# wildminder/ComfyUI-KEEP

Hardware: AMD Instinct MI355X
Metric: restored 512x512 face frames/sec, T=20 clip (higher is better)
Workload: dtype f16x3; 1 GPU; 48 independent clips x T=20 x 512x512 per GPU (BASELINE configs[1] clips), KEEP config, synthetic weights seed 0, precision policy x3; clips_per_gpu=48, clip_length=20, parallelism=dp1 over clips, precision_policy=x3

## Files before the change

### comfyui-keep_amd/csrc/keep_attn.hip

```cpp
#include <math.h>
#include <stdlib.h>

#include <type_traits>

#include "keep_common.h"
#include "../../include/keep_cv_hip.h"

static constexpr int KEEP_NT_ATTN_O = 0;


struct AttnP {
  const float* q;
  const float* k;
  const float* v;
  const unsigned short* q16;
  const unsigned short* k16;
  const unsigned short* v16;
  float* o;
  long q_bs, q_ts, q_hs, k_bs, k_ts, k_hs, v_bs, v_ts, v_hs, o_bs, o_ts, o_hs;
  int B, H, Lq, Lk, D, Dv;
  float scale;
  int mode, T, seg_len;
  int img_h, img_w, ksplit, shift, kv_rot, n_img;
  int nslices;
// ... 235 lines not shown
        if (t < p.Lk) kreg[u] = *reinterpret_cast<const float4*>(p.k + kv_offset(p, b, t, p.k_bs, p.k_ts) + kh + c);
      }
      if (i < 32 * vc4n) {
        const int row = i / vc4n, c = (i - row * vc4n) << 2;
        const int t = kt * 32 + row;
        if (t < p.Lk && dv0 + c < p.Dv)
          vreg[u] = *reinterpret_cast<const float4*>(p.v + kv_offset(p, b, t, p.v_bs, p.v_ts) + vh + dv0 + c);
      }
    }
  };
  auto pf_commit = [&]() {
#pragma unroll
    for (int u = 0; u < PF; ++u) {
      const int i = tid + u * NT;
      if (i < 32 * kc4n) {
        const int row = i / kc4n, c = (i - row * kc4n) << 2;
        float* d = Ks + row * QP + c;
        d[0] = kreg[u].x; d[1] = kreg[u].y; d[2] = kreg[u].z; d[3] = kreg[u].w;
      }
      if (i < 32 * vc4n) {
        const int row = i / vc4n, c = (i - row * vc4n) << 2;
        *reinterpret_cast<float4*>(Vs + row * DVS + c) = vreg[u];
      }
    }
  };

  if (prefetch) {
    pf_issue(0);
    pf_commit();
  }

  for (int kt = 0; kt < ntiles; ++kt) {
    f32x16 s;
#pragma unroll
    for (int r = 0; r < 16; ++r) s[r] = 0.f;

    if (prefetch) {
      __syncthreads();
      if (kt + 1 < ntiles) pf_issue(kt + 1);
      for (int d2 = 0; d2 < DC; d2 += 2) s = __builtin_amdgcn_mfma_f32_32x32x2f32(kp[d2], qp[d2], s, 0, 0, 0);
    } else {
      for (int ch = 0; ch < nch; ++ch) {
        __syncthreads();
        if (nch > 1)
          load_tile_direct<NT, true>(p, p.q, p.q_bs, p.q_ts, qh, b, q0, p.Lq, WAVES * 32, ch * DC, DC, p.D, Qs, QP,
                                     tid, qk_vec);
        load_tile_direct<NT, false>(p, p.k, p.k_bs, p.k_ts, kh, b, kt * 32, p.Lk, 32, ch * DC, DC, p.D, Ks, QP, tid,
                                    qk_vec);
        if (ch == 0)
          load_tile_direct<NT, false>(p, p.v, p.v_bs, p.v_ts, vh, b, kt * 32, p.Lk, 32, dv0, DVS, p.Dv, Vs, DVS, tid,
                                      v_vec);
        __syncthreads();
        for (int d2 = 0; d2 < DC; d2 += 2) s = __builtin_amdgcn_mfma_f32_32x32x2f32(kp[d2], qp[d2], s, 0, 0, 0);
      }
    }

    float mloc = -INFINITY;
#pragma unroll
    for (int r = 0; r < 16; ++r) {
      const int key = kt * 32 + (r & 3) + 8 * (r >> 2) + 4 * lhi;
      float val = s[r] * p.scale;
      if (p.mode == 2 && p.shift > 0 && key < p.Lk) {
        if (win_region(p, b, key) != my_region) val += -100.0f;
      }
      if (key >= p.Lk) val = -INFINITY;
      s[r] = val;
      mloc = fmaxf(mloc, val);
    }
    mloc = fmaxf(mloc, __shfl_xor(mloc, 32));
    const float m_new = fmaxf(m_run, mloc);
    const float alpha = expf(m_run - m_new);
    float lsum = 0.f;
#pragma unroll
    for (int r = 0; r < 16; ++r) {
      const float pv = expf(s[r] - m_new);
      s[r] = pv;
      lsum += pv;
    }
    lsum += __shfl_xor(lsum, 32);
    l_run = l_run * alpha + lsum;
    m_run = m_new;

#pragma unroll
    for (int r = 0; r < 16; ++r) {
      const int qrow = (r & 3) + 8 * (r >> 2) + 4 * lhi;
      const float ar = __shfl(alpha, qrow);
#pragma unroll
      for (int j = 0; j < DVT; ++j) o[j][r] *= ar;
    }
#pragma unroll
    for (int r = 0; r < 16; ++r) {
      const int krow = (r & 3) + 8 * (r >> 2) + 4 * lhi;
      const float* vp = Vs + krow * DVS + l31;
#pragma unroll
      for (int j = 0; j < DVT; ++j) o[j] = __builtin_amdgcn_mfma_f32_32x32x2f32(s[r], vp[j * 32], o[j], 0, 0, 0);
    }
    if (prefetch && kt + 1 < ntiles) {
      __syncthreads();
      pf_commit();
    }
  }

  const float inv_l = 1.0f / l_run;
#pragma unroll
  for (int r = 0; r < 16; ++r) {
    const int qrow = (r & 3) + 8 * (r >> 2) + 4 * lhi;
    const float il = __shfl(inv_l, qrow);
    const int t = q0 + wave * 32 + qrow;
    if (t < p.Lq) {
      const long base = q_offset(p, b, t, p.o_bs, p.o_ts) + (long)head * p.o_hs;
#pragma unroll
      for (int j = 0; j < DVT; ++j) {
        const int dv = dv0 + j * 32 + l31;
        if (dv < p.Dv) p.o[base + dv] = o[j][r] * il;
      }
    }
  }
}

template <int WAVES, int DVT>
static int launch_attn(const AttnP& p, const AttnPlan& pl, hipStream_t st) {
  const int rc = keep_raise_lds_limit<attn_f32_kernel<WAVES, DVT>>("keep_attention");
  if (rc != KEEP_OK) return rc;
  dim3 grid(cdiv(p.Lq, WAVES * 32), p.H * p.nslices, p.B);
  hipLaunchKernelGGL((attn_f32_kernel<WAVES, DVT>), grid, dim3(64 * WAVES), pl.lds, st, p);
  KEEP_LAUNCH_CHECK("keep_attention");
  return KEEP_OK;
}

typedef __attribute__((ext_vector_type(8))) __bf16 abf16x8;

__device__ __forceinline__ int vt_pos(int key) {
  return (((key >> 4) << 1) + ((key >> 2) & 1)) * 8 + ((((key >> 3) & 1) << 2) | (key & 3));
}

template <int WAVES, int DVT>
__global__ __launch_bounds__(64 * WAVES) void attn_bf16_kernel(AttnP p) {
  extern __shared__ __attribute__((aligned(16))) __bf16 smem16[];
  constexpr int DVS = DVT * 32;
  constexpr int NT = 64 * WAVES;
  constexpr int VP = 40;
  const int DC = p.D < 128 ? p.D : 128;
  const int nch = p.D / DC;
  const int QP = DC + 8;
  __bf16* Qs = smem16;
  __bf16* Ks = Qs + WAVES * 32 * QP;
  __bf16* Vt = Ks + 32 * QP;

  const int tid = threadIdx.x;
  const int lane = tid & 63;
  const int wave = tid >> 6;
  const int l31 = lane & 31, lhi = lane >> 5;
  const int b = blockIdx.z;
  const int head = blockIdx.y / p.nslices;
  const int dv0 = (blockIdx.y - head * p.nslices) * DVS;
  const int q0 = blockIdx.x * (WAVES * 32);
  const long qh = (long)head * p.q_hs, kh = (long)head * p.k_hs, vh = (long)head * p.v_hs;
  const int g8n = DC >> 3;

  auto stage_rows = [&](const float* base, long bs, long ts, long hoff, bool is_q, int t0, int tmax, int nrows,
                        int c0, __bf16* dst) {
    for (int i = tid; i < nrows * g8n; i += NT) {
      const int row = i / g8n, c = (i - row * g8n) << 3;
      const int t = t0 + row;
      abf16x8 h;
      if (t < tmax) {
        const float* src = base + (is_q ? q_offset(p, b, t, bs, ts) : kv_offset(p, b, t, bs, ts)) + hoff + c0 + c;
        const float4 a = *reinterpret_cast<const float4*>(src);
        const float4 c4 = *reinterpret_cast<const float4*>(src + 4);
        h[0] = (__bf16)a.x; h[1] = (__bf16)a.y; h[2] = (__bf16)a.z; h[3] = (__bf16)a.w;
        h[4] = (__bf16)c4.x; h[5] = (__bf16)c4.y; h[6] = (__bf16)c4.z; h[7] = (__bf16)c4.w;
      } else {
#pragma unroll
        for (int j = 0; j < 8; ++j) h[j] = (__bf16)0.f;
      }
      *reinterpret_cast<abf16x8*>(dst + row * QP + c) = h;
    }
  };
  auto stage_vt = [&](int kt) {
    for (int i = tid; i < 16 * DVS; i += NT) {
      const int pair = i / DVS, dv = i - pair * DVS;
      const int k0 = pair * 2;
      const int t = kt * 32 + k0;
      float v0 = 0.f, v1 = 0.f;
      if (dv0 + dv < p.Dv) {
        if (t < p.Lk) v0 = p.v[kv_offset(p, b, t, p.v_bs, p.v_ts) + vh + dv0 + dv];
        if (t + 1 < p.Lk) v1 = p.v[kv_offset(p, b, t + 1, p.v_bs, p.v_ts) + vh + dv0 + dv];
      }
      __bf16* d = Vt + dv * VP + vt_pos(k0);
      d[0] = (__bf16)v0;
      d[1] = (__bf16)v1;
    }
  };

  if (nch == 1) stage_rows(p.q, p.q_bs, p.q_ts, qh, true, q0, p.Lq, WAVES * 32, 0, Qs);

  const int my_q = q0 + wave * 32 + l31;
  int my_region = 0;
  if (p.mode == 2 && p.shift > 0 && my_q < p.Lq) my_region = win_region(p, b, my_q);

  float m_run = -INFINITY, l_run = 0.f;
  f32x16 o[DVT];
#pragma unroll
  for (int j = 0; j < DVT; ++j)
#pragma unroll
    for (int r = 0; r < 16; ++r) o[j][r] = 0.f;

  const __bf16* kp = Ks + l31 * QP + lhi * 8;
  const __bf16* qp = Qs + (wave * 32 + l31) * QP + lhi * 8;
  const int ntiles = (p.Lk + 31) / 32;

  for (int kt = 0; kt < ntiles; ++kt) {
    f32x16 s;
#pragma unroll
    for (int r = 0; r < 16; ++r) s[r] = 0.f;
    for (int ch = 0; ch < nch; ++ch) {
      __syncthreads();
      if (nch > 1) stage_rows(p.q, p.q_bs, p.q_ts, qh, true, q0, p.Lq, WAVES * 32, ch * DC, Qs);
      stage_rows(p.k, p.k_bs, p.k_ts, kh, false, kt * 32, p.Lk, 32, ch * DC, Ks);
      if (ch == 0) stage_vt(kt);
      __syncthreads();
      for (int d = 0; d < DC; d += 16)
        s = __builtin_amdgcn_mfma_f32_32x32x16_bf16(*reinterpret_cast<const abf16x8*>(kp + d),
                                                    *reinterpret_cast<const abf16x8*>(qp + d), s, 0, 0, 0);
    }

    float mloc = -INFINITY;
#pragma unroll
    for (int r = 0; r < 16; ++r) {
      const int key = kt * 32 + (r & 3) + 8 * (r >> 2) + 4 * lhi;
      float val = s[r] * p.scale;
      if (p.mode == 2 && p.shift > 0 && key < p.Lk) {
        if (win_region(p, b, key) != my_region) val += -100.0f;
      }
      if (key >= p.Lk) val = -INFINITY;
      s[r] = val;
      mloc = fmaxf(mloc, val);
    }
    mloc = fmaxf(mloc, __shfl_xor(mloc, 32));
    const float m_new = fmaxf(m_run, mloc);
    const float alpha = __expf(m_run - m_new);
    float lsum = 0.f;
#pragma unroll
    for (int r = 0; r < 16; ++r) {
      const float pv = __expf(s[r] - m_new);
      s[r] = pv;
      lsum += pv;
    }
    lsum += __shfl_xor(lsum, 32);
    l_run = l_run * alpha + lsum;
    m_run = m_new;

#pragma unroll
    for (int r = 0; r < 16; ++r) {
      const int qrow = (r & 3) + 8 * (r >> 2) + 4 * lhi;
      const float ar = __shfl(alpha, qrow);
#pragma unroll
      for (int j = 0; j < DVT; ++j) o[j][r] *= ar;
    }
#pragma unroll
    for (int st = 0; st < 2; ++st) {
      abf16x8 pa;
#pragma unroll
      for (int j = 0; j < 8; ++j) pa[j] = (__bf16)s[st * 8 + j];
#pragma unroll
      for (int j = 0; j < DVT; ++j) {
        const abf16x8 vb = *reinterpret_cast<const abf16x8*>(Vt + (j * 32 + l31) * VP + (st * 2 + lhi) * 8);
        o[j] = __builtin_amdgcn_mfma_f32_32x32x16_bf16(pa, vb, o[j], 0, 0, 0);
      }
    }
  }

  const float inv_l = 1.0f / l_run;
#pragma unroll
  for (int r = 0; r < 16; ++r) {
    const int qrow = (r & 3) + 8 * (r >> 2) + 4 * lhi;
    const float il = __shfl(inv_l, qrow);
    const int t = q0 + wave * 32 + qrow;
    if (t < p.Lq) {
      const long base = q_offset(p, b, t, p.o_bs, p.o_ts) + (long)head * p.o_hs;
#pragma unroll
      for (int j = 0; j < DVT; ++j) {
        const int dv = dv0 + j * 32 + l31;
        if (dv < p.Dv) p.o[base + dv] = o[j][r] * il;
      }
    }
  }
}

template <int WAVES, int DVT>
static int launch_attn_bf16(const AttnP& p, const AttnPlan& pl, hipStream_t st) {
  const int rc = keep_raise_lds_limit<attn_bf16_kernel<WAVES, DVT>>("keep_attention");
  if (rc != KEEP_OK) return rc;
  dim3 grid(cdiv(p.Lq, WAVES * 32), p.H * p.nslices, p.B);
  hipLaunchKernelGGL((attn_bf16_kernel<WAVES, DVT>), grid, dim3(64 * WAVES), pl.lds, st, p);
  KEEP_LAUNCH_CHECK("keep_attention(bf16)");
  return KEEP_OK;
}

typedef _Float16 af16x8 __attribute__((ext_vector_type(8)));
typedef _Float16 af16x4 __attribute__((ext_vector_type(4)));
typedef _Float16 af16x2 __attribute__((ext_vector_type(2)));

template <int WAVES, int DVT, int NQ, bool PACKED = false, bool X1 = false>
__global__ __launch_bounds__(64 * WAVES, ((WAVES == 4 && NQ != 16) ? 2 : 1)) void attn_x3_kernel(AttnP p) {
  static_assert(!X1 || (PACKED && WAVES == 4 && NQ == 8), "the single-fp16 form exists for the packed D = 128 kernel only");
  constexpr bool QREG = NQ > 0;
  constexpr int NQA = QREG ? NQ : 1;
  extern __shared__ __attribute__((aligned(16))) _Float16 smemx[];
  constexpr int DVS = DVT * 32;
  constexpr int NT = 64 * WAVES;
  constexpr int VP = X1 ? 40 : 72;
  constexpr bool PF = (WAVES == 4) && QREG;
  constexpr int KPF = PF ? (32 * 4 * NQA + NT - 1) / NT : 1;
  constexpr int VPF = PF ? (16 * DVS + NT - 1) / NT : 1;
  const int DCMAX = QREG ? 16 * NQA : 128;
  const int DC = p.D < DCMAX ? p.D : DCMAX;
  const int nch = p.D / DC;
  const int QP = (X1 ? DC : 2 * DC) + 8;
  _Float16* Ks = smemx;
  _Float16* Vt = Ks + 32 * QP;
  _Float16* Qs = Vt + DVS * VP;
  const bool tab = PF && p.mode == 2 && p.Lk <= 4096;
  int* tpix = reinterpret_cast<int*>(Qs);
  unsigned* treg = reinterpret_cast<unsigned*>(tpix + ((p.Lk + 31) & ~31));

  const int tid = threadIdx.x;
  const int lane = tid & 63;
  const int wave = tid >> 6;
  const int l31 = lane & 31, lhi = lane >> 5;
  int bx = blockIdx.x, by = blockIdx.y, bz = blockIdx.z;
  {
    const int gx = gridDim.x, gy = gridDim.y, total = gx * gy * gridDim.z;
    const int lid = bx + gx * (by + gy * bz);
    const int qd = total >> 3, rm = total & 7, xcd = lid & 7, slot = lid >> 3;
    const int logical = (xcd < rm ? xcd * (qd + 1) : rm * (qd + 1) + (xcd - rm) * qd) + slot;
    bx = logical % gx;
    const int rest = logical / gx;
    by = rest % gy;
    bz = rest / gy;
  }
  const int b = bz;
  const int head = by / p.nslices;
  const int dv0 = (by - head * p.nslices) * DVS;
  const int q0 = bx * (WAVES * 32);
  const long qh = (long)head * p.q_hs, kh = (long)head * p.k_hs, vh = (long)head * p.v_hs;
  const int g4n = DC >> 2;
  WinCtx wc;
  if (tab) {
    wc = win_ctx(p, b);
    const int ntl = (p.Lk + 31) >> 5;
    unsigned char* treg8 = reinterpret_cast<unsigned char*>(treg + ntl * 4);
    for (int t = tid; t < ntl * 32; t += NT) {
      int pix = 0, region = 0;
      if (t < p.Lk) win_token(p, wc, t, pix, region);
      tpix[t] = pix;
      treg8[t] = (unsigned char)region;
    }
    __syncthreads();
    for (int i = tid; i < ntl * 4; i += NT) {
      unsigned w = 0;
#pragma unroll
      for (int j = 0; j < 8; ++j) w |= (unsigned)treg8[i * 8 + j] << (4 * j);
      treg[i] = w;
    }
    __syncthreads();
  }
  float sq = 1.f, sk = 1.f, sv = 1.f, inv_qk = 1.f, inv_sv = 1.f;
  if (p.q_amax) {
    float iq, ik;
    attn_range_scale(p.q_amax[b], sq, iq);
    attn_range_scale(p.k_amax[b], sk, ik);
    attn_range_scale(p.v_amax[b], sv, inv_sv);
    inv_qk = iq * ik;
  }

  auto split8 = [&](const float4 a, const float4 c, float sc, af16x8& hi, af16x8& lo) {
    const float f[8] = {a.x * sc, a.y * sc, a.z * sc, a.w * sc, c.x * sc, c.y * sc, c.z * sc, c.w * sc};
#pragma unroll
    for (int j = 0; j < 8; ++j) {
      const _Float16 h = (_Float16)f[j];
      hi[j] = h;
      lo[j] = (_Float16)(f[j] - (float)h);
    }
  };
  auto split_store4 = [&](const float4 v, float sc, _Float16* dst) {
    const float f[4] = {v.x * sc, v.y * sc, v.z * sc, v.w * sc};
    af16x4 hi, lo;
#pragma unroll
    for (int j = 0; j < 4; ++j) {
      const _Float16 h = (_Float16)f[j];
      hi[j] = h;
      lo[j] = (_Float16)(f[j] - (float)h);
    }
    *reinterpret_cast<af16x4*>(dst) = hi;
    *reinterpret_cast<af16x4*>(dst + DC) = lo;
  };
  auto stage_rows = [&](const float* base, long bs, long ts, long hoff, bool is_q, int t0, int tmax, int nrows, int c0,
                        _Float16* dst) {
    for (int i = tid; i < nrows * g4n; i += NT) {
      const int row = i / g4n, c = (i - row * g4n) << 2;
      const int t = t0 + row;
      float4 v = make_float4(0.f, 0.f, 0.f, 0.f);
      if (t < tmax)
        v = *reinterpret_cast<const float4*>(base + (is_q ? q_offset(p, b, t, bs, ts) : kv_offset(p, b, t, bs, ts)) + hoff + c0 + c);
      split_store4(v, is_q ? sq : sk, dst + row * QP + c);
    }
  };
  auto stage_vt = [&](int kt) {
    for (int i = tid; i < 16 * DVS; i += NT) {
      const int pair = i / DVS, dv = i - pair * DVS;
      const int t = kt * 32 + pair * 2;
      float v[2] = {0.f, 0.f};
      if (dv0 + dv < p.Dv) {
        if (t < p.Lk) v[0] = p.v[kv_offset(p, b, t, p.v_bs, p.v_ts) + vh + dv0 + dv];
        if (t + 1 < p.Lk) v[1] = p.v[kv_offset(p, b, t + 1, p.v_bs, p.v_ts) + vh + dv0 + dv];
      }
      af16x2 hi, lo;
#pragma unroll
      for (int j = 0; j < 2; ++j) {
        const float vs = v[j] * sv;
        const _Float16 h = (_Float16)vs;
        hi[j] = h;
        lo[j] = (_Float16)(vs - (float)h);
      }
      _Float16* d = Vt + dv * VP + vt_pos(pair * 2);
      *reinterpret_cast<af16x2*>(d) = hi;
      *reinterpret_cast<af16x2*>(d + 32) = lo;
    }
  };
  float4 kreg[KPF];
  float vreg[VPF][2];
  auto k_issue = [&](int kt) {
#pragma unroll
    for (int u = 0; u < KPF; ++u) {
      const int i = tid + u * NT;
      kreg[u] = make_float4(0.f, 0.f, 0.f, 0.f);
      if (i < 32 * g4n) {
        const int row = i / g4n, c = (i - row * g4n) << 2;
        const int t = kt * 32 + row;
        if (t < p.Lk) {
          const long off = tab ? (long)wc.img_kv * p.k_bs + (long)tpix[t] * p.k_ts : kv_offset(p, b, t, p.k_bs, p.k_ts);
          kreg[u] = *reinterpret_cast<const float4*>(p.k + off + kh + c);
        }
      }
    }
  };
  auto k_commit = [&]() {
#pragma unroll
    for (int u = 0; u < KPF; ++u) {
      const int i = tid + u * NT;
      if (i < 32 * g4n) {
        const int row = i / g4n, c = (i - row * g4n) << 2;
        split_store4(kreg[u], sk, Ks + row * QP + c);
      }
    }
  };
  auto v_issue = [&](int kt) {
#pragma unroll
    for (int u = 0; u < VPF; ++u) {
      const int i = tid + u * NT;
      vreg[u][0] = 0.f;
      vreg[u][1] = 0.f;
      if (i < 16 * DVS) {
        const int pair = i / DVS, dv = i - pair * DVS;
        const int t = kt * 32 + pair * 2;
        if (dv0 + dv < p.Dv) {
          if (tab) {
            const long vb = (long)wc.img_kv * p.v_bs + vh + dv0 + dv;
            if (t < p.Lk) vreg[u][0] = p.v[vb + (long)tpix[t] * p.v_ts];
            if (t + 1 < p.Lk) vreg[u][1] = p.v[vb + (long)tpix[t + 1] * p.v_ts];
          } else {
            if (t < p.Lk) vreg[u][0] = p.v[kv_offset(p, b, t, p.v_bs, p.v_ts) + vh + dv0 + dv];
            if (t + 1 < p.Lk) vreg[u][1] = p.v[kv_offset(p, b, t + 1, p.v_bs, p.v_ts) + vh + dv0 + dv];
          }
        }
      }
    }
  };
  auto v_commit = [&]() {
#pragma unroll
    for (int u = 0; u < VPF; ++u) {
      const int i = tid + u * NT;
      if (i < 16 * DVS) {
        const int pair = i / DVS, dv = i - pair * DVS;
        af16x2 hi, lo;
#pragma unroll
        for (int j = 0; j < 2; ++j) {
          const float vs = vreg[u][j] * sv;
          const _Float16 h = (_Float16)vs;
          hi[j] = h;
          lo[j] = (_Float16)(vs - (float)h);
        }
        _Float16* d = Vt + dv * VP + vt_pos(pair * 2);
        *reinterpret_cast<af16x2*>(d) = hi;
        *reinterpret_cast<af16x2*>(d + 32) = lo;
      }
    }
  };

  constexpr int PKK = PACKED ? 32 * ((X1 ? 1 : 2) * 16 * NQA + 8) / 8 : 1;
  constexpr int PKV = PACKED ? DVS * VP / 8 : 1;
  constexpr int PK16 = PKK + PKV;
  constexpr int PKN = PACKED ? (PK16 + NT - 1) / NT : 1;
  uint4 preg[PKN];
  auto pk_issue = [&](int kt) {
    const long tile = ((long)b * p.H + head) * ((p.Lk + 31) >> 5) + kt;
    const uint4* src = reinterpret_cast<const uint4*>(p.kv_pack) + tile * (PKK + p.nslices * PKV);
    const int vs = PKK + (dv0 / DVS) * PKV;
#pragma unroll
    for (int u = 0; u < PKN; ++u) {
      const int i = tid + u * NT;
      preg[u] = make_uint4(0u, 0u, 0u, 0u);
      if (i < PK16) preg[u] = src[i < PKK ? i : vs + (i - PKK)];
    }
  };
  auto pk_commit = [&]() {
#pragma unroll
    for (int u = 0; u < PKN; ++u) {
      const int i = tid + u * NT;
      if (i < PK16) reinterpret_cast<uint4*>(Ks)[i] = preg[u];
    }
  };

  const int my_q = q0 + wave * 32 + l31;
  af16x8 qfh[NQA], qfl[NQA];
  if (QREG) {
    const bool qok = my_q < p.Lq;
    const float* qrow = p.q + (qok ? q_offset(p, b, my_q, p.q_bs, p.q_ts) + qh : 0) + lhi * 8;
#pragma unroll
    for (int d8 = 0; d8 < NQA; ++d8) {
      float4 a = make_float4(0.f, 0.f, 0.f, 0.f), c = a;
      if (qok && d8 * 16 < DC) {
        a = *reinterpret_cast<const float4*>(qrow + d8 * 16);
        c = *reinterpret_cast<const float4*>(qrow + d8 * 16 + 4);
      }
      split8(a, c, sq, qfh[QREG ? d8 : 0], qfl[QREG ? d8 : 0]);
    }
  }
  if (PF) {
    if (PACKED) {
      pk_issue(0);
      pk_commit();
    } else {
      k_issue(0);
      v_issue(0);
      k_commit();
      v_commit();
    }
  }

  int my_region = 0;
  if (p.mode == 2 && p.shift > 0 && my_q < p.Lq) my_region = win_region(p, b, my_q);

  const float qk_scale = p.scale * inv_qk;
  const float qk_scale2 = qk_scale * 1.4426950408889634f;
  float m_run = -INFINITY, l_run = 0.f;
  f32x16 o[DVT];
#pragma unroll
  for (int j = 0; j < DVT; ++j)
#pragma unroll
    for (int r = 0; r < 16; ++r) o[j][r] = 0.f;

  const _Float16* kp = Ks + l31 * QP + lhi * 8;
  const _Float16* qp = Qs + (wave * 32 + l31) * QP + lhi * 8;
  const int ntiles = (p.Lk + 31) / 32;

  for (int kt = 0; kt < ntiles; ++kt) {
    f32x16 s;
#pragma unroll
    for (int r = 0; r < 16; ++r) s[r] = 0.f;
    if (QREG) {
      if (!PF) {
        __syncthreads();
        stage_rows(p.k, p.k_bs, p.k_ts, kh, false, kt * 32, p.Lk, 32, 0, Ks);
        stage_vt(kt);
      }
      __syncthreads();
      if (PF && kt + 1 < ntiles) {
        if (PACKED) {
          pk_issue(kt + 1);
        } else {
          k_issue(kt + 1);
          v_issue(kt + 1);
        }
      }
#pragma unroll
      for (int d8 = 0; d8 < NQA; ++d8) {
        if (d8 * 16 < DC) {
          const af16x8 kh8 = *reinterpret_cast<const af16x8*>(kp + d8 * 16);
          if (!X1) {
            const af16x8 kl8 = *reinterpret_cast<const af16x8*>(kp + DC + d8 * 16);
            s = __builtin_amdgcn_mfma_f32_32x32x16_f16(kl8, qfh[QREG ? d8 : 0], s, 0, 0, 0);
            s = __builtin_amdgcn_mfma_f32_32x32x16_f16(kh8, qfl[QREG ? d8 : 0], s, 0, 0, 0);
          }
          s = __builtin_amdgcn_mfma_f32_32x32x16_f16(kh8, qfh[QREG ? d8 : 0], s, 0, 0, 0);
        }
      }
    } else {
      for (int ch = 0; ch < nch; ++ch) {
        __syncthreads();
        stage_rows(p.q, p.q_bs, p.q_ts, qh, true, q0, p.Lq, WAVES * 32, ch * DC, Qs);
        stage_rows(p.k, p.k_bs, p.k_ts, kh, false, kt * 32, p.Lk, 32, ch * DC, Ks);
        if (ch == 0) stage_vt(kt);
        __syncthreads();
        for (int d = 0; d < DC; d += 16) {
          const af16x8 kh8 = *reinterpret_cast<const af16x8*>(kp + d), kl8 = *reinterpret_cast<const af16x8*>(kp + DC + d);
          const af16x8 qh8 = *reinterpret_cast<const af16x8*>(qp + d), ql8 = *reinterpret_cast<const af16x8*>(qp + DC + d);
          s = __builtin_amdgcn_mfma_f32_32x32x16_f16(kl8, qh8, s, 0, 0, 0);
          s = __builtin_amdgcn_mfma_f32_32x32x16_f16(kh8, ql8, s, 0, 0, 0);
          s = __builtin_amdgcn_mfma_f32_32x32x16_f16(kh8, qh8, s, 0, 0, 0);
        }
      }
    }

    float mloc = -INFINITY;
    if (PF) {
      uint4 rw = make_uint4(0u, 0u, 0u, 0u);
      const bool masked = p.mode == 2 && p.shift > 0;
      if (masked && tab) rw = *reinterpret_cast<const uint4*>(treg + kt * 4);
      const unsigned rws[4] = {rw.x, rw.y, rw.z, rw.w};
#pragma unroll
      for (int r = 0; r < 16; ++r) {
        const int kl = (r & 3) + 8 * (r >> 2) + 4 * lhi;
        const int key = kt * 32 + kl;
        float val = s[r] * qk_scale2;
        if (masked) {
          const int kr = tab ? (int)((rws[r >> 2] >> (4 * ((r & 3) + 4 * lhi))) & 15u) : (key < p.Lk ? win_region(p, b, key) : my_region);
          if (kr != my_region) val += -100.0f * 1.4426950408889634f;
        }
        if (key >= p.Lk) val = -INFINITY;
        s[r] = val;
        mloc = fmaxf(mloc, val);
      }
    } else {
#pragma unroll
      for (int r = 0; r < 16; ++r) {
        const int key = kt * 32 + (r & 3) + 8 * (r >> 2) + 4 * lhi;
        float val = s[r] * qk_scale;
        if (p.mode == 2 && p.shift > 0 && key < p.Lk) {
          if (win_region(p, b, key) != my_region) val += -100.0f;
        }
        if (key >= p.Lk) val = -INFINITY;
        s[r] = val;
        mloc = fmaxf(mloc, val);
      }
    }
    mloc = fmaxf(mloc, __shfl_xor(mloc, 32));
    const float m_new = fmaxf(m_run, mloc);
    const float alpha = PF ? __builtin_amdgcn_exp2f(m_run - m_new) : expf(m_run - m_new);
    float lsum = 0.f;
#pragma unroll
    for (int r = 0; r < 16; ++r) {
      const float pv = PF ? __builtin_amdgcn_exp2f(s[r] - m_new) : expf(s[r] - m_new);
      s[r] = pv;
      lsum += pv;
    }
    lsum += __shfl_xor(lsum, 32);
    l_run = l_run * alpha + lsum;
    m_run = m_new;

    if (!PF || __builtin_amdgcn_ballot_w64(alpha != 1.0f) != 0ull) {
#pragma unroll
      for (int r = 0; r < 16; ++r) {
        const int qrow = (r & 3) + 8 * (r >> 2) + 4 * lhi;
        const float ar = __shfl(alpha, qrow);
#pragma unroll
        for (int j = 0; j < DVT; ++j) o[j][r] *= ar;
      }
    }
#pragma unroll
    for (int st = 0; st < 2; ++st) {
      af16x8 ph, pl;
#pragma unroll
      for (int j = 0; j < 8; ++j) {
        const _Float16 h = (_Float16)s[st * 8 + j];
        ph[j] = h;
        pl[j] = (_Float16)(s[st * 8 + j] - (float)h);
      }
#pragma unroll
      for (int j = 0; j < DVT; ++j) {
        const _Float16* vrow = Vt + (j * 32 + l31) * VP + (st * 2 + lhi) * 8;
        const af16x8 vh8 = *reinterpret_cast<const af16x8*>(vrow);
        if (!X1) {
          const af16x8 vl8 = *reinterpret_cast<const af16x8*>(vrow + 32);
          o[j] = __builtin_amdgcn_mfma_f32_32x32x16_f16(pl, vh8, o[j], 0, 0, 0);
          o[j] = __builtin_amdgcn_mfma_f32_32x32x16_f16(ph, vl8, o[j], 0, 0, 0);
        }
        o[j] = __builtin_amdgcn_mfma_f32_32x32x16_f16(ph, vh8, o[j], 0, 0, 0);
      }
    }
    if (PF && kt + 1 < ntiles) {
      __syncthreads();
      if (PACKED) {
        pk_commit();
      } else {
        k_commit();
        v_commit();
      }
    }
  }

  const float inv_l = inv_sv / l_run;
#pragma unroll
  for (int r = 0; r < 16; ++r) {
    const int qrow = (r & 3) + 8 * (r >> 2) + 4 * lhi;
    const float il = __shfl(inv_l, qrow);
    const int t = q0 + wave * 32 + qrow;
    if (t < p.Lq) {
      const long base = q_offset(p, b, t, p.o_bs, p.o_ts) + (long)head * p.o_hs;
#pragma unroll
      for (int j = 0; j < DVT; ++j) {
        const int dv = dv0 + j * 32 + l31;
        if (dv >= p.Dv) continue;
        if (KEEP_NT_ATTN_O)
          __builtin_nontemporal_store(o[j][r] * il, p.o + base + dv);
        else
          p.o[base + dv] = o[j][r] * il;
      }
    }
  }
}

template <int DC, int DVS, bool X1 = false>
__global__ __launch_bounds__(256) void attn_pack_kv_x3_kernel(AttnP p, _Float16* out) {
  constexpr int QP = (X1 ? DC : 2 * DC) + 8, VP = X1 ? 40 : 72, PKK = 32 * QP / 8, PKV = DVS * VP / 8;
  __shared__ __attribute__((aligned(16))) _Float16 img[32 * QP + DVS * VP];
  _Float16* Ks = img;
  _Float16* Vt = img + 32 * QP;
  const int tid = threadIdx.x;
  const int kt = blockIdx.x, head = blockIdx.y / p.nslices, slice = blockIdx.y - head * p.nslices, b = blockIdx.z;
  float sk = 1.f, sv = 1.f, tmp;
  if (p.q_amax) {
    attn_range_scale(p.k_amax[b], sk, tmp);
    attn_range_scale(p.v_amax[b], sv, tmp);
  }
  for (int i = tid; i < PKK + PKV; i += 256) reinterpret_cast<uint4*>(img)[i] = make_uint4(0u, 0u, 0u, 0u);
  __syncthreads();
  const long kh = (long)head * p.k_hs, vh = (long)head * p.v_hs;
  if (slice == 0) {
    for (int i = tid; i < 32 * (DC / 4); i += 256) {
      const int row = i / (DC / 4), c = (i - row * (DC / 4)) << 2;
      const int t = kt * 32 + row;
      if (t < p.Lk) {
        const float4 v = *reinterpret_cast<const float4*>(p.k + kv_offset(p, b, t, p.k_bs, p.k_ts) + kh + c);
        const float f[4] = {v.x * sk, v.y * sk, v.z * sk, v.w * sk};
        af16x4 hi, lo;
#pragma unroll
        for (int j = 0; j < 4; ++j) {
          const _Float16 h = (_Float16)f[j];
          hi[j] = h;
          lo[j] = (_Float16)(f[j] - (float)h);
        }
        *reinterpret_cast<af16x4*>(Ks + row * QP + c) = hi;
        if (!X1) *reinterpret_cast<af16x4*>(Ks + row * QP + DC + c) = lo;
      }
    }
  }
  const int dv0 = slice * DVS;
  for (int i = tid; i < 16 * DVS; i += 256) {
    const int pair = i / DVS, dv = i - pair * DVS;
    const int t = kt * 32 + pair * 2;
    float v[2] = {0.f, 0.f};
    if (dv0 + dv < p.Dv) {
      if (t < p.Lk) v[0] = p.v[kv_offset(p, b, t, p.v_bs, p.v_ts) + vh + dv0 + dv];
      if (t + 1 < p.Lk) v[1] = p.v[kv_offset(p, b, t + 1, p.v_bs, p.v_ts) + vh + dv0 + dv];
    }
    af16x2 hi, lo;
#pragma unroll
    for (int j = 0; j < 2; ++j) {
      const float vs = v[j] * sv;
      const _Float16 h = (_Float16)vs;
      hi[j] = h;
      lo[j] = (_Float16)(vs - (float)h);
    }
    _Float16* d = Vt + dv * VP + vt_pos(pair * 2);
    *reinterpret_cast<af16x2*>(d) = hi;
    if (!X1) *reinterpret_cast<af16x2*>(d + 32) = lo;
  }
  __syncthreads();
  uint4* dst = reinterpret_cast<uint4*>(out) + (((long)b * p.H + head) * gridDim.x + kt) * (PKK + p.nslices * PKV);
  if (slice == 0)
    for (int i = tid; i < PKK; i += 256) dst[i] = reinterpret_cast<const uint4*>(img)[i];
  for (int i = tid; i < PKV; i += 256) dst[PKK + slice * PKV + i] = reinterpret_cast<const uint4*>(img)[PKK + i];
}

template <int DVT, int NQ, bool X1 = false>
static int launch_attn_x3_packed(const AttnP& p, const AttnPlan& pl, hipStream_t st) {
  const int ntl = (p.Lk + 31) / 32;
  hipLaunchKernelGGL((attn_pack_kv_x3_kernel<16 * NQ, DVT * 32, X1>), dim3(ntl, p.H * p.nslices, p.B), dim3(256), 0, st, p,
                     const_cast<_Float16*>(p.kv_pack));
  KEEP_LAUNCH_CHECK("keep_attention(x3 pack)");
  const int rc = keep_raise_lds_limit<attn_x3_kernel<4, DVT, NQ, true, X1>>("keep_attention");
  if (rc != KEEP_OK) return rc;
  dim3 grid(cdiv(p.Lq, 128), p.H * p.nslices, p.B);
  hipLaunchKernelGGL((attn_x3_kernel<4, DVT, NQ, true, X1>), grid, dim3(256), pl.lds, st, p);
  KEEP_LAUNCH_CHECK("keep_attention(x3 packed)");
  return KEEP_OK;
}

template <int WAVES, int DVT, int NQ>
static int launch_attn_x3_t(const AttnP& p, const AttnPlan& pl, hipStream_t st) {
  const int rc = keep_raise_lds_limit<attn_x3_kernel<WAVES, DVT, NQ>>("keep_attention");
  if (rc != KEEP_OK) return rc;
  dim3 grid(cdiv(p.Lq, WAVES * 32), p.H * p.nslices, p.B);
  hipLaunchKernelGGL((attn_x3_kernel<WAVES, DVT, NQ>), grid, dim3(64 * WAVES), pl.lds, st, p);
  KEEP_LAUNCH_CHECK("keep_attention(x3)");
  return KEEP_OK;
}

template <int DVT>
__global__ __launch_bounds__(256, 1) void attn_x3_sfull_kernel(AttnP p) {
  extern __shared__ __attribute__((aligned(16))) _Float16 smemx[];
  constexpr int DVS = DVT * 32, NT = 256, VP = 72, DC = 128, QP = 2 * DC + 8, KT2 = 64;
  _Float16* Qs = smemx;
  _Float16* Ks = Qs + 128 * QP;
  _Float16* Vt = Ks + KT2 * QP;
  const int tid = threadIdx.x;
  const int lane = tid & 63;
  const int wave = tid >> 6;
  const int l31 = lane & 31, lhi = lane >> 5;
  const int b = blockIdx.z;
  const int head = blockIdx.y / p.nslices;
  const int dv0 = (blockIdx.y - head * p.nslices) * DVS;
  const int q0 = blockIdx.x * 128;
  const long qh = (long)head * p.q_hs, kh = (long)head * p.k_hs, vh = (long)head * p.v_hs;
  const int nch = p.D / DC;
  const int ntiles = (p.Lk + 31) / 32;
  float sq = 1.f, sk = 1.f, sv = 1.f, inv_qk = 1.f, inv_sv = 1.f;
  if (p.q_amax) {
    float iq, ik;
    attn_range_scale(p.q_amax[b], sq, iq);
    attn_range_scale(p.k_amax[b], sk, ik);
    attn_range_scale(p.v_amax[b], sv, inv_sv);
    inv_qk = iq * ik;
  }
  auto stage_rows = [&](const float* base, long bs, long ts, long hoff, int t0, int tmax, int nrows, int c0, float sc, _Float16* dst) {
    for (int i = tid; i < nrows * (DC / 4); i += NT) {
      const int row = i / (DC / 4), c = (i - row * (DC / 4)) << 2;
      const int t = t0 + row;
      float4 v = make_float4(0.f, 0.f, 0.f, 0.f);
      if (t < tmax) v = *reinterpret_cast<const float4*>(base + (long)b * bs + (long)t * ts + hoff + c0 + c);
      const float f[4] = {v.x * sc, v.y * sc, v.z * sc, v.w * sc};
      af16x4 hi, lo;
#pragma unroll
      for (int j = 0; j < 4; ++j) {
        const _Float16 h = (_Float16)f[j];
        hi[j] = h;
        lo[j] = (_Float16)(f[j] - (float)h);
      }
      *reinterpret_cast<af16x4*>(dst + row * QP + c) = hi;
      *reinterpret_cast<af16x4*>(dst + row * QP + c + DC) = lo;
    }
  };
  f32x16 s[8];
#pragma unroll
  for (int k = 0; k < 8; ++k)
#pragma unroll
    for (int r = 0; r < 16; ++r) s[k][r] = 0.f;
  const _Float16* qp = Qs + (wave * 32 + l31) * QP + lhi * 8;
  for (int ch = 0; ch < nch; ++ch) {
    __syncthreads();
    stage_rows(p.q, p.q_bs, p.q_ts, qh, q0, p.Lq, 128, ch * DC, sq, Qs);
#pragma unroll
    for (int k2 = 0; k2 < 4; ++k2) {
      if (k2 * 2 < ntiles) {
        if (k2 > 0) __syncthreads();
        stage_rows(p.k, p.k_bs, p.k_ts, kh, k2 * KT2, p.Lk, KT2, ch * DC, sk, Ks);
        __syncthreads();
#pragma unroll
        for (int d = 0; d < DC; d += 16) {
          const af16x8 qh8 = *reinterpret_cast<const af16x8*>(qp + d), ql8 = *reinterpret_cast<const af16x8*>(qp + DC + d);
#pragma unroll
          for (int t = 0; t < 2; ++t) {
            const _Float16* kp = Ks + (t * 32 + l31) * QP + lhi * 8 + d;
            const af16x8 kh8 = *reinterpret_cast<const af16x8*>(kp), kl8 = *reinterpret_cast<const af16x8*>(kp + DC);
            s[k2 * 2 + t] = __builtin_amdgcn_mfma_f32_32x32x16_f16(kl8, qh8, s[k2 * 2 + t], 0, 0, 0);
            s[k2 * 2 + t] = __builtin_amdgcn_mfma_f32_32x32x16_f16(kh8, ql8, s[k2 * 2 + t], 0, 0, 0);
            s[k2 * 2 + t] = __builtin_amdgcn_mfma_f32_32x32x16_f16(kh8, qh8, s[k2 * 2 + t], 0, 0, 0);
          }
        }
      }
    }
  }
  const float qk_scale = p.scale * inv_qk;
  float m = -INFINITY;
#pragma unroll
  for (int k = 0; k < 8; ++k)
#pragma unroll
    for (int r = 0; r < 16; ++r) {
      const int key = k * 32 + (r & 3) + 8 * (r >> 2) + 4 * lhi;
      const float val = key < p.Lk ? s[k][r] * qk_scale : -INFINITY;
      s[k][r] = val;
      m = fmaxf(m, val);
    }
  m = fmaxf(m, __shfl_xor(m, 32));
  float lsum = 0.f;
#pragma unroll
  for (int k = 0; k < 8; ++k)
#pragma unroll
    for (int r = 0; r < 16; ++r) {
      const float pv = expf(s[k][r] - m);
      s[k][r] = pv;
      lsum += pv;
    }
  lsum += __shfl_xor(lsum, 32);
  f32x16 o[DVT];
#pragma unroll
  for (int j = 0; j < DVT; ++j)
#pragma unroll
    for (int r = 0; r < 16; ++r) o[j][r] = 0.f;
#pragma unroll
  for (int kt = 0; kt < 8; ++kt) {
    if (kt < ntiles) {
      __syncthreads();
      for (int i = tid; i < 16 * DVS; i += NT) {
        const int pair = i / DVS, dv = i - pair * DVS;
        const int t = kt * 32 + pair * 2;
        float v[2] = {0.f, 0.f};
        if (dv0 + dv < p.Dv) {
          if (t < p.Lk) v[0] = p.v[(long)b * p.v_bs + (long)t * p.v_ts + vh + dv0 + dv];
          if (t + 1 < p.Lk) v[1] = p.v[(long)b * p.v_bs + (long)(t + 1) * p.v_ts + vh + dv0 + dv];
        }
        af16x2 hi, lo;
#pragma unroll
        for (int j = 0; j < 2; ++j) {
          const float vs = v[j] * sv;
          const _Float16 h = (_Float16)vs;
          hi[j] = h;
          lo[j] = (_Float16)(vs - (float)h);
        }
        _Float16* d = Vt + dv * VP + vt_pos(pair * 2);
        *reinterpret_cast<af16x2*>(d) = hi;
        *reinterpret_cast<af16x2*>(d + 32) = lo;
      }
      __syncthreads();
#pragma unroll
      for (int st = 0; st < 2; ++st) {
        af16x8 ph, pl;
#pragma unroll
        for (int j = 0; j < 8; ++j) {
          const _Float16 h = (_Float16)s[kt][st * 8 + j];
          ph[j] = h;
          pl[j] = (_Float16)(s[kt][st * 8 + j] - (float)h);
        }
#pragma unroll
        for (int j = 0; j < DVT; ++j) {
          const _Float16* vrow = Vt + (j * 32 + l31) * VP + (st * 2 + lhi) * 8;
          const af16x8 vh8 = *reinterpret_cast<const af16x8*>(vrow), vl8 = *reinterpret_cast<const af16x8*>(vrow + 32);
          o[j] = __builtin_amdgcn_mfma_f32_32x32x16_f16(pl, vh8, o[j], 0, 0, 0);
          o[j] = __builtin_amdgcn_mfma_f32_32x32x16_f16(ph, vl8, o[j], 0, 0, 0);
          o[j] = __builtin_amdgcn_mfma_f32_32x32x16_f16(ph, vh8, o[j], 0, 0, 0);
        }
      }
    }
  }
  const float inv_l = inv_sv / lsum;
#pragma unroll
  for (int r = 0; r < 16; ++r) {
    const int qrow = (r & 3) + 8 * (r >> 2) + 4 * lhi;
    const float il = __shfl(inv_l, qrow);
    const int t = q0 + wave * 32 + qrow;
    if (t < p.Lq) {
      const long base = (long)b * p.o_bs + (long)t * p.o_ts + (long)head * p.o_hs;
#pragma unroll
      for (int j = 0; j < DVT; ++j) {
        const int dv = dv0 + j * 32 + l31;
        if (dv < p.Dv) p.o[base + dv] = o[j][r] * il;
      }
    }
  }
}

__global__ __launch_bounds__(256, 1) void attn_x3_sfull2_kernel(AttnP p) {
  extern __shared__ __attribute__((aligned(16))) _Float16 smemx[];
  constexpr int DC = 128, QP = 2 * DC + 8, VP = 72, DVS = 128;
  constexpr int WREG = 2 * 32 * QP;
  static_assert(WREG >= DVS * VP, "V^T tile fits the wave's staging region");
  const int tid = threadIdx.x;
  const int lane = tid & 63;
  const int wave = tid >> 6;
  const int l31 = lane & 31, lhi = lane >> 5;
  const int b = blockIdx.z, head = blockIdx.y, q0 = blockIdx.x * 32;
  _Float16* Qw = smemx + wave * WREG;
  _Float16* Kw = Qw + 32 * QP;
  _Float16* Vt = Qw;
  float* red = reinterpret_cast<float*>(smemx + 4 * WREG);
  const long qh = (long)head * p.q_hs, kh = (long)head * p.k_hs, vh = (long)head * p.v_hs;
  const int ntiles = (p.Lk + 31) / 32;
  float sq = 1.f, sk = 1.f, sv = 1.f, inv_qk = 1.f, inv_sv = 1.f;
  if (p.q_amax) {
    float iq, ik;
    attn_range_scale(p.q_amax[b], sq, iq);
    attn_range_scale(p.k_amax[b], sk, ik);
    attn_range_scale(p.v_amax[b], sv, inv_sv);
    inv_qk = iq * ik;
  }
  float4 buf[16];
  auto load_rows = [&](const float* base, long bs, long ts, long hoff, int t0, int tmax) {
#pragma unroll
    for (int u = 0; u < 16; ++u) {
      const int i = lane + u * 64;
      const int row = i >> 5, c = (i & 31) << 2;
      const int t = t0 + row;
      buf[u] = make_float4(0.f, 0.f, 0.f, 0.f);
      if (t < tmax) buf[u] = *reinterpret_cast<const float4*>(base + (long)b * bs + (long)t * ts + hoff + wave * DC + c);
    }
  };
  auto split_rows = [&](float sc, _Float16* dst) {
#pragma unroll
    for (int u = 0; u < 16; ++u) {
      const int i = lane + u * 64;
      const int row = i >> 5, c = (i & 31) << 2;
      const float f[4] = {buf[u].x * sc, buf[u].y * sc, buf[u].z * sc, buf[u].w * sc};
      af16x4 hi, lo;
#pragma unroll
      for (int j = 0; j < 4; ++j) {
        const _Float16 h = (_Float16)f[j];
        hi[j] = h;
        lo[j] = (_Float16)(f[j] - (float)h);
      }
      *reinterpret_cast<af16x4*>(dst + row * QP + c) = hi;
      *reinterpret_cast<af16x4*>(dst + row * QP + c + DC) = lo;
// ... 1381 lines not shown
```

Measured before the change: 297.1 frames/s.

## Specialise packed x3 attention kernel on launch-constant mask modes and peel last tile

Splits the x3 attention kernel into a body template specialised on mask and table flags, which are read once at kernel entry, and peels the final key tile so the steady-state loop skips prefetch and bounds checks. It also software-pipelines the K fragment LDS loads and hoists the V fragment loads ahead of the MFMA chains. Per-row shuffles become readlane broadcasts, and the region-mask test becomes a precomputed XOR. Together these cut per-tile scalar and branch work in the packed path, at the cost of four instantiations per config, which adds code size and may change register pressure.

```diff
diff --git a/comfyui-keep_amd/csrc/keep_attn.hip b/comfyui-keep_amd/csrc/keep_attn.hip
--- a/comfyui-keep_amd/csrc/keep_attn.hip
+++ b/comfyui-keep_amd/csrc/keep_attn.hip
@@ -561,9 +561,11 @@
 typedef _Float16 af16x4 __attribute__((ext_vector_type(4)));
 typedef _Float16 af16x2 __attribute__((ext_vector_type(2)));
 
-template <int WAVES, int DVT, int NQ, bool PACKED = false, bool X1 = false>
-__global__ __launch_bounds__(64 * WAVES, ((WAVES == 4 && NQ != 16) ? 2 : 1)) void attn_x3_kernel(AttnP p) {
+template <int WAVES, int DVT, int NQ, bool PACKED, bool X1, int MT>
+__device__ __forceinline__ void attn_x3_body(const AttnP& p) {
   static_assert(!X1 || (PACKED && WAVES == 4 && NQ == 8), "the single-fp16 form exists for the packed D = 128 kernel only");
+  static_assert(MT < 0 || PACKED, "the launch-constant loop exists for the packed forms");
+  constexpr bool SPEC = MT >= 0;
   constexpr bool QREG = NQ > 0;
   constexpr int NQA = QREG ? NQ : 1;
   extern __shared__ __attribute__((aligned(16))) _Float16 smemx[];
@@ -574,17 +576,19 @@
   constexpr int KPF = PF ? (32 * 4 * NQA + NT - 1) / NT : 1;
   constexpr int VPF = PF ? (16 * DVS + NT - 1) / NT : 1;
   const int DCMAX = QREG ? 16 * NQA : 128;
-  const int DC = p.D < DCMAX ? p.D : DCMAX;
-  const int nch = p.D / DC;
+  const int DC = SPEC ? 16 * NQA : (p.D < DCMAX ? p.D : DCMAX);
+  const int nch = SPEC ? 1 : p.D / DC;
   const int QP = (X1 ? DC : 2 * DC) + 8;
   _Float16* Ks = smemx;
   _Float16* Vt = Ks + 32 * QP;
   _Float16* Qs = Vt + DVS * VP;
-  const bool tab = PF && p.mode == 2 && p.Lk <= 4096;
+  const bool tab = SPEC ? (MT & 2) != 0 : (PF && p.mode == 2 && p.Lk <= 4096);
+  const bool masked = SPEC ? (MT & 1) != 0 : (p.mode == 2 && p.shift > 0);
   int* tpix = reinterpret_cast<int*>(Qs);
   unsigned* treg = reinterpret_cast<unsigned*>(tpix + ((p.Lk + 31) & ~31));
 
   const int tid = threadIdx.x;
+  __builtin_assume(tid < NT);
   const int lane = tid & 63;
   const int wave = tid >> 6;
   const int l31 = lane & 31, lhi = lane >> 5;
@@ -765,13 +769,14 @@
   uint4 preg[PKN];
   auto pk_issue = [&](int kt) {
     const long tile = ((long)b * p.H + head) * ((p.Lk + 31) >> 5) + kt;
-    const uint4* src = reinterpret_cast<const uint4*>(p.kv_pack) + tile * (PKK + p.nslices * PKV);
-    const int vs = PKK + (dv0 / DVS) * PKV;
+    const char* src = reinterpret_cast<const char*>(p.kv_pack) + tile * (PKK + p.nslices * PKV) * 16;
+    const unsigned t16 = (unsigned)tid * 16u, vsh = (unsigned)(dv0 / DVS) * (unsigned)(PKV * 16);
 #pragma unroll
     for (int u = 0; u < PKN; ++u) {
       const int i = tid + u * NT;
       preg[u] = make_uint4(0u, 0u, 0u, 0u);
-      if (i < PK16) preg[u] = src[i < PKK ? i : vs + (i - PKK)];
+      const unsigned off = t16 + ((u + 1) * NT <= PKK ? 0u : (u * NT >= PKK || i >= PKK ? vsh : 0u));
+      if (i < PK16) preg[u] = *reinterpret_cast<const uint4*>(src + u * NT * 16 + off);
     }
   };
   auto pk_commit = [&]() {
@@ -825,7 +830,16 @@
   const _Float16* qp = Qs + (wave * 32 + l31) * QP + lhi * 8;
   const int ntiles = (p.Lk + 31) / 32;
 
-  for (int kt = 0; kt < ntiles; ++kt) {
+  auto row_bcast = [&](const float x, const int r) {
+    const int q0 = (r & 3) + 8 * (r >> 2);
+    const float a0 = __int_as_float(__builtin_amdgcn_readlane(__float_as_int(x), q0));
+    const float a1 = __int_as_float(__builtin_amdgcn_readlane(__float_as_int(x), q0 + 4));
+    return lhi ? a1 : a0;
+  };
+
+  auto tile = [&](const int kt, auto tmc) {
+    constexpr int TM = decltype(tmc)::value;
+    const bool more = TM == 0 ? true : (TM == 1 ? false : kt + 1 < ntiles);
     f32x16 s;
 #pragma unroll
     for (int r = 0; r < 16; ++r) s[r] = 0.f;
@@ -836,7 +850,7 @@
         stage_vt(kt);
       }
       __syncthreads();
-      if (PF && kt + 1 < ntiles) {
+      if (PF && more) {
         if (PACKED) {
           pk_issue(kt + 1);
         } else {
@@ -844,16 +858,35 @@
           v_issue(kt + 1);
         }
       }
-#pragma unroll
-      for (int d8 = 0; d8 < NQA; ++d8) {
-        if (d8 * 16 < DC) {
-          const af16x8 kh8 = *reinterpret_cast<const af16x8*>(kp + d8 * 16);
+      if (SPEC) {
+        af16x8 kh8[2], kl8[2];
+        kh8[0] = *reinterpret_cast<const af16x8*>(kp);
+        if (!X1) kl8[0] = *reinterpret_cast<const af16x8*>(kp + DC);
+#pragma unroll
+        for (int d8 = 0; d8 < NQA; ++d8) {
+          const int c = d8 & 1;
+          if (d8 + 1 < NQA) {
+            kh8[c ^ 1] = *reinterpret_cast<const af16x8*>(kp + (d8 + 1) * 16);
+            if (!X1) kl8[c ^ 1] = *reinterpret_cast<const af16x8*>(kp + DC + (d8 + 1) * 16);
+          }
           if (!X1) {
-            const af16x8 kl8 = *reinterpret_cast<const af16x8*>(kp + DC + d8 * 16);
-            s = __builtin_amdgcn_mfma_f32_32x32x16_f16(kl8, qfh[QREG ? d8 : 0], s, 0, 0, 0);
-            s = __builtin_amdgcn_mfma_f32_32x32x16_f16(kh8, qfl[QREG ? d8 : 0], s, 0, 0, 0);
+            s = __builtin_amdgcn_mfma_f32_32x32x16_f16(kl8[c], qfh[d8], s, 0, 0, 0);
+            s = __builtin_amdgcn_mfma_f32_32x32x16_f16(kh8[c], qfl[d8], s, 0, 0, 0);
           }
-          s = __builtin_amdgcn_mfma_f32_32x32x16_f16(kh8, qfh[QREG ? d8 : 0], s, 0, 0, 0);
+          s = __builtin_amdgcn_mfma_f32_32x32x16_f16(kh8[c], qfh[d8], s, 0, 0, 0);
+        }
+      } else {
+#pragma unroll
+        for (int d8 = 0; d8 < NQA; ++d8) {
+          if (d8 * 16 < DC) {
+            const af16x8 kh8 = *reinterpret_cast<const af16x8*>(kp + d8 * 16);
+            if (!X1) {
+              const af16x8 kl8 = *reinterpret_cast<const af16x8*>(kp + DC + d8 * 16);
+              s = __builtin_amdgcn_mfma_f32_32x32x16_f16(kl8, qfh[QREG ? d8 : 0], s, 0, 0, 0);
+              s = __builtin_amdgcn_mfma_f32_32x32x16_f16(kh8, qfl[QREG ? d8 : 0], s, 0, 0, 0);
+            }
+            s = __builtin_amdgcn_mfma_f32_32x32x16_f16(kh8, qfh[QREG ? d8 : 0], s, 0, 0, 0);
+          }
         }
       }
     } else {
@@ -876,19 +909,21 @@
     float mloc = -INFINITY;
     if (PF) {
       uint4 rw = make_uint4(0u, 0u, 0u, 0u);
-      const bool masked = p.mode == 2 && p.shift > 0;
       if (masked && tab) rw = *reinterpret_cast<const uint4*>(treg + kt * 4);
-      const unsigned rws[4] = {rw.x, rw.y, rw.z, rw.w};
+      const unsigned mine = (unsigned)my_region * 0x1111u;
+      const unsigned rws[4] = {((rw.x >> (16 * lhi)) & 0xffffu) ^ mine, ((rw.y >> (16 * lhi)) & 0xffffu) ^ mine,
+                               ((rw.z >> (16 * lhi)) & 0xffffu) ^ mine, ((rw.w >> (16 * lhi)) & 0xffffu) ^ mine};
 #pragma unroll
       for (int r = 0; r < 16; ++r) {
         const int kl = (r & 3) + 8 * (r >> 2) + 4 * lhi;
         const int key = kt * 32 + kl;
         float val = s[r] * qk_scale2;
+        if (SPEC) asm volatile("" : "+v"(val));
         if (masked) {
-          const int kr = tab ? (int)((rws[r >> 2] >> (4 * ((r & 3) + 4 * lhi))) & 15u) : (key < p.Lk ? win_region(p, b, key) : my_region);
-          if (kr != my_region) val += -100.0f * 1.4426950408889634f;
+          const bool cross = tab ? (rws[r >> 2] & (15u << (4 * (r & 3)))) != 0u : (key < p.Lk ? win_region(p, b, key) : my_region) != my_region;
+          if (cross) val += -100.0f * 1.4426950408889634f;
         }
-        if (key >= p.Lk) val = -INFINITY;
+        if (TM != 0 && key >= p.Lk) val = -INFINITY;
         s[r] = val;
         mloc = fmaxf(mloc, val);
       }
@@ -916,20 +951,26 @@
       lsum += pv;
     }
     lsum += __shfl_xor(lsum, 32);
-    l_run = l_run * alpha + lsum;
+    l_run = __builtin_fmaf(l_run, alpha, lsum);
     m_run = m_new;
 
     if (!PF || __builtin_amdgcn_ballot_w64(alpha != 1.0f) != 0ull) {
 #pragma unroll
       for (int r = 0; r < 16; ++r) {
-        const int qrow = (r & 3) + 8 * (r >> 2) + 4 * lhi;
-        const float ar = __shfl(alpha, qrow);
+        const float ar = row_bcast(alpha, r);
 #pragma unroll
         for (int j = 0; j < DVT; ++j) o[j][r] *= ar;
       }
     }
 #pragma unroll
     for (int st = 0; st < 2; ++st) {
+      af16x8 vh8[DVT], vl8[DVT];
+#pragma unroll
+      for (int j = 0; j < DVT; ++j) {
+        const _Float16* vrow = Vt + (j * 32 + l31) * VP + (st * 2 + lhi) * 8;
+        vh8[j] = *reinterpret_cast<const af16x8*>(vrow);
+        if (!X1) vl8[j] = *reinterpret_cast<const af16x8*>(vrow + 32);
+      }
       af16x8 ph, pl;
 #pragma unroll
       for (int j = 0; j < 8; ++j) {
@@ -937,19 +978,16 @@
         ph[j] = h;
         pl[j] = (_Float16)(s[st * 8 + j] - (float)h);
       }
-#pragma unroll
-      for (int j = 0; j < DVT; ++j) {
-        const _Float16* vrow = Vt + (j * 32 + l31) * VP + (st * 2 + lhi) * 8;
-        const af16x8 vh8 = *reinterpret_cast<const af16x8*>(vrow);
-        if (!X1) {
-          const af16x8 vl8 = *reinterpret_cast<const af16x8*>(vrow + 32);
-          o[j] = __builtin_amdgcn_mfma_f32_32x32x16_f16(pl, vh8, o[j], 0, 0, 0);
-          o[j] = __builtin_amdgcn_mfma_f32_32x32x16_f16(ph, vl8, o[j], 0, 0, 0);
-        }
-        o[j] = __builtin_amdgcn_mfma_f32_32x32x16_f16(ph, vh8, o[j], 0, 0, 0);
-      }
-    }
-    if (PF && kt + 1 < ntiles) {
+      if (!X1) {
+#pragma unroll
+        for (int j = 0; j < DVT; ++j) o[j] = __builtin_amdgcn_mfma_f32_32x32x16_f16(pl, vh8[j], o[j], 0, 0, 0);
+#pragma unroll
+        for (int j = 0; j < DVT; ++j) o[j] = __builtin_amdgcn_mfma_f32_32x32x16_f16(ph, vl8[j], o[j], 0, 0, 0);
+      }
+#pragma unroll
+      for (int j = 0; j < DVT; ++j) o[j] = __builtin_amdgcn_mfma_f32_32x32x16_f16(ph, vh8[j], o[j], 0, 0, 0);
+    }
+    if (PF && more) {
       __syncthreads();
       if (PACKED) {
         pk_commit();
@@ -958,13 +996,19 @@
         v_commit();
       }
     }
+  };
+  if (SPEC) {
+    for (int kt = 0; kt + 1 < ntiles; ++kt) tile(kt, std::integral_constant<int, 0>{});
+    tile(ntiles - 1, std::integral_constant<int, 1>{});
+  } else {
+    for (int kt = 0; kt < ntiles; ++kt) tile(kt, std::integral_constant<int, 2>{});
   }
 
   const float inv_l = inv_sv / l_run;
 #pragma unroll
   for (int r = 0; r < 16; ++r) {
     const int qrow = (r & 3) + 8 * (r >> 2) + 4 * lhi;
-    const float il = __shfl(inv_l, qrow);
+    const float il = row_bcast(inv_l, r);
     const int t = q0 + wave * 32 + qrow;
     if (t < p.Lq) {
       const long base = q_offset(p, b, t, p.o_bs, p.o_ts) + (long)head * p.o_hs;
@@ -978,6 +1022,26 @@
           p.o[base + dv] = o[j][r] * il;
       }
     }
+  }
+}
+
+template <int WAVES, int DVT, int NQ, bool PACKED = false, bool X1 = false>
+__global__ __launch_bounds__(64 * WAVES, ((WAVES == 4 && NQ != 16) ? 2 : 1)) void attn_x3_kernel(AttnP p) {
+  if constexpr (PACKED) {
+    const bool masked = p.mode == 2 && p.shift > 0, tab = p.mode == 2 && p.Lk <= 4096;
+    if (masked) {
+      if (tab)
+        attn_x3_body<WAVES, DVT, NQ, PACKED, X1, 3>(p);
+      else
+        attn_x3_body<WAVES, DVT, NQ, PACKED, X1, 1>(p);
+    } else {
+      if (tab)
+        attn_x3_body<WAVES, DVT, NQ, PACKED, X1, 2>(p);
+      else
+        attn_x3_body<WAVES, DVT, NQ, PACKED, X1, 0>(p);
+    }
+  } else {
+    attn_x3_body<WAVES, DVT, NQ, PACKED, X1, -1>(p);
   }
 }
 
```

Result: no change. 299.6 frames/s, median of 6 (+0.8%).
